# mahdeslami11/jalil-saboorizadeh-Multi-speaker-Neural-Vocoder

Measured on AMD Instinct MI355X. Metric: audio samples/sec gen (3-tier dim1024) + TBPTT steps/sec @1/2/4/8 GPU, higher is better.
Workload: dtype bf16

## Files before the change

### jalil-saboorizadeh-multi-speaker-neural-vocoder_amd/csrc/gru_xcd.hip

```cpp
#include <algorithm>

#include "samplernn_hip_internal.hpp"
#include "handoff.hpp"
#include "gru_point.hpp"

namespace gx {
constexpr int NW = 8, NTHR = NW * 64;
constexpr int RG = 16;
constexpr int CU = 32;
constexpr int NT = 6;
constexpr int UK = 32;
constexpr int MAXMT = 4;
constexpr int PS = 68;
constexpr int HDR = 2048;
}

__device__ __forceinline__ void gx_note_failure(const int* err, int* sticky) {
    if (threadIdx.x == 0) {
        const int e = __hip_atomic_load(err, __ATOMIC_RELAXED, __HIP_MEMORY_SCOPE_AGENT);
        if (e) __hip_atomic_fetch_max(sticky, e, __ATOMIC_RELAXED, __HIP_MEMORY_SCOPE_AGENT);
    }
}

struct GruXArgs {
    const float* gi; int64_t ldgi; int64_t sgi;
    const float* h0;
    const bf16* whh; const float* bhh;
    float* out; bf16* out_lp; int64_t ldo; int64_t so;
    bf16* hp_lp;
    float* gates; int64_t ldg; int64_t sg;
    u64* xh;
    int* census;
    int nolocal;
    int* err;
    int* sticky;
    int spin_limit;
    int withhold;
    int B, D, Fr, G, P, RV;
    int poll_sleep;
    unsigned long long* diag;
    int exp;
};

template <int UPW, int MT, int DC = 0>
__global__ __launch_bounds__(gx::NTHR, 2) void gru_xcd_fwd_kernel(GruXArgs a) {
    using namespace gx;
    extern __shared__ __attribute__((aligned(16))) char smem[];
    const int tid = threadIdx.x, wave = tid >> 6, lane = tid & 63;
    const int D = DC ? DC : a.D, B = a.B, RV = a.RV;
    const int NU = D / UK, KW = NW < NU ? NW : NU;
    float* red = (float*)smem;
    int* gsh = (int*)(smem + (size_t)2 * KW * NT * 4 * PS * sizeof(float));
    const int g = blockIdx.x % a.G, p = blockIdx.x / a.G;
    if (tid == 0) hx_group_arrive(a.census + g * a.P + p);
    const int u0 = p * CU;
    const int DG = D / 2;
    unsigned long long* dg = (a.diag && blockIdx.x == 0 && tid == 0) ? a.diag : nullptr;
    int nd = 0;
#define GX_STAMP() do { if (dg && nd < 255) dg[nd++] = __builtin_amdgcn_s_memrealtime(); } while (0)
    bf16x8 wf[UPW][NT];
    {
        const int PW = 2 * D + 16;
        const int PPR = D / 8;
        char* stg = smem;
        uint4 lw[UPW][NT];
#pragma unroll
        for (int gate = 0; gate < 3; ++gate) {
            if (gate) __syncthreads();
            const bf16* src = a.whh + (int64_t)(gate * D + u0) * D;
            if constexpr (DC != 0) {
                constexpr int NPT = 32 * (DC / 8) / NTHR;
                uint4 v[NPT];
#pragma unroll
                for (int i = 0; i < NPT; ++i) {
                    const int e = tid + i * NTHR, rr = e / PPR, c = e - rr * PPR;
                    v[i] = *reinterpret_cast<const uint4*>(src + (int64_t)rr * D + c * 8);
                }
#pragma unroll
                for (int i = 0; i < NPT; ++i) {
                    const int e = tid + i * NTHR, rr = e / PPR, c = e - rr * PPR;
                    *reinterpret_cast<uint4*>(stg + rr * PW + c * 16) = v[i];
                }
            } else {
                for (int e = tid; e < 32 * PPR; e += NTHR) {
                    const int rr = e / PPR, c = e - rr * PPR;
                    *reinterpret_cast<uint4*>(stg + rr * PW + c * 16) =
                        *reinterpret_cast<const uint4*>(src + (int64_t)rr * D + c * 8);
                }
            }
            __syncthreads();
#pragma unroll
            for (int j = 0; j < UPW; ++j) {
                const int u = wave + NW * j;
                const int ke = min(u * UK + (lane >> 4) * 8, D - 8);
#pragma unroll
                for (int h = 0; h < 2; ++h)
                    lw[j][2 * gate + h] = *reinterpret_cast<const uint4*>(
                        stg + (h * 16 + (lane & 15)) * PW + ke * 2);
            }
        }
        __syncthreads();
#pragma unroll
        for (int j = 0; j < UPW; ++j) {
            const bool kv = wave + NW * j < NU;
#pragma unroll
            for (int t = 0; t < NT; ++t) {
                const uint4 v = kv ? lw[j][t] : make_uint4(0u, 0u, 0u, 0u);
                __builtin_memcpy(&wf[j][t], &v, 16);
            }
        }
    }
    if (wave == 0) {
        const int loc = hx_group_local(a.census + g * a.P, a.P, a.err, !a.nolocal) ? 1 : 0;
        if (tid == 0) gsh[2] = loc;
    }
    __syncthreads();
    const bool local = gsh[2] != 0;
    if (dg) dg[255] = local ? 1 : 2;
    const int r = tid >> 5, uu = tid & 31;
    const bool rv = r < RV;
    const int unit = u0 + uu;
    int rop = r;
    auto row_of = [&](int m) { return (g * MT + m) * RV + rop; };
    const float bhr = a.bhh[unit], bhz = a.bhh[D + unit], bhn = a.bhh[2 * D + unit];
    float hprev[MT];
#pragma unroll
    for (int m = 0; m < MT; ++m) {
        const int row = row_of(m);
        const int b = min(row, B - 1);
        hprev[m] = a.h0[(int64_t)b * D + unit];
        if (a.hp_lp && rv && row < B)
            a.hp_lp[(int64_t)b * a.ldo + unit] = __float2bfloat16(hprev[m]);
    }
    const __amdgpu_buffer_rsrc_t rx = hx_rsrc(a.xh);
    const size_t bufw = (size_t)a.G * MT * RG * DG;
    auto publish = [&](int s, int m, float h) {
        const uint32_t mine = (uint32_t)__bfloat16_as_ushort(__float2bfloat16(h));
        const uint32_t nb = lane_next16(mine);
        if ((uu & 1) == 0 && !(a.withhold && blockIdx.x == 0))
            hx_put(a.xh + ((s + 1) & 1) * bufw + (size_t)(g * MT + m) * RG * DG +
                       ((size_t)(((unit >> 5) * 2 + ((unit & 7) >> 2)) * 64 +
                                 ((unit & 31) >> 3) * 16 + r) << 1) + ((unit & 3) >> 1),
                   (uint32_t)(s + 2), mine | (nb << 16), local);
    };
#pragma unroll
    for (int m = 0; m < MT; ++m) publish(-1, m, hprev[m]);
    const int lrow = lane & 15;
    struct Gi { float r, z, n; };
    Gi ga, gb{0.f, 0.f, 0.f};
    const bool ntl = !(a.exp & 512), nts = !(a.exp & 2048);
    auto ld = [ntl](const float* p) { return ntl ? __builtin_nontemporal_load(p) : *p; };
    {
        const float* gp0 = a.gi + (int64_t)min(row_of(0), B - 1) * a.ldgi;
        ga = Gi{ld(gp0 + unit), ld(gp0 + D + unit), ld(gp0 + 2 * D + unit)};
    }
    auto fetch_gi = [&](int t, int m, Gi& nx) {
        if (a.exp & 2) return;
        int tn = t, mn = m + 1;
        if (mn == MT) { mn = 0; tn = min(t + 1, a.Fr - 1); }
        const float* gp = a.gi + (int64_t)min(row_of(mn), B - 1) * a.ldgi + (int64_t)tn * a.sgi;
        nx.r = ld(gp + unit); nx.z = ld(gp + D + unit); nx.n = ld(gp + 2 * D + unit);
    };
    auto step = [&](int t, int m, const Gi& cu, Gi& nx) {
            floatx4 acc[NT];
    #pragma unroll
            for (int i = 0; i < NT; ++i) acc[i] = floatx4{0.f, 0.f, 0.f, 0.f};
            const bool polls = UPW >= 2 || wave < KW;
            if (!polls) fetch_gi(t, m, nx);
            if (polls) {
                const uint32_t tag = (uint32_t)(t + 1);
                const uint32_t base = (uint32_t)(((size_t)(t & 1) * bufw +
                                                  (size_t)(g * MT + m) * RG * DG) * 8) +
                                      (lrow < RV ? lane * 16u : 0x80000000u);
                uint32_t w[UPW][4];
                int spins = 0;
                for (;;) {
                    uint4 x[UPW][2];
    #pragma unroll
                    for (int j = 0; j < UPW; ++j) {
                        const int u = min(wave + NW * j, NU - 1);
                        const uint32_t off = base + (uint32_t)u * 2048u;
                        x[j][0] = hx_get2(rx, off);
                        x[j][1] = hx_get2(rx, off + 1024);
                    }
                    bool ok = true;
    #pragma unroll
                    for (int j = 0; j < UPW; ++j) {
                        const bool v = wave + NW * j < NU;
                        w[j][0] = v ? x[j][0].x : 0u; w[j][1] = v ? x[j][0].z : 0u;
                        w[j][2] = v ? x[j][1].x : 0u; w[j][3] = v ? x[j][1].z : 0u;
                        ok &= !v || ((x[j][0].y == tag) & (x[j][0].w == tag) &
                                     (x[j][1].y == tag) & (x[j][1].w == tag));
                    }
                    ok |= lrow >= RV;
                    if (__all(ok)) break;
                    if (hx_spin_fail(spins, a.err, lane, a.poll_sleep, a.spin_limit)) break;
                }
                fetch_gi(t, m, nx);
                GX_STAMP();
    #pragma unroll
                for (int j = 0; j < UPW; ++j) {
                    const uint4 v = make_uint4(w[j][0], w[j][1], w[j][2], w[j][3]);
                    bf16x8 af;
                    __builtin_memcpy(&af, &v, 16);
    #pragma unroll
                    for (int i = 0; i < NT; ++i) Mma<bf16>::run(acc[i], af, wf[j][i]);
                }
                float* rb = red + (size_t)(((t * MT + m) & 1) * KW + wave) * NT * 4 * PS + lane;
    #pragma unroll
                for (int i = 0; i < NT; ++i)
    #pragma unroll
                    for (int e = 0; e < 4; ++e) rb[(i * 4 + e) * PS] = acc[i][e];
            }
            GX_STAMP();
            __syncthreads();
            GX_STAMP();
            float gh[3];
            {
                const int ln = (r >> 2) * 16 + (uu & 15), ii = r & 3;
                const float* rb = red + (size_t)((t * MT + m) & 1) * KW * NT * 4 * PS + ii * PS + ln;
    #pragma unroll
                for (int gt = 0; gt < 3; ++gt) {
                    const int tile = 2 * gt + (uu >> 4);
                    float v = 0.f;
                    float pr[NW];
                    #pragma unroll
                    for (int kw = 0; kw < NW; ++kw)
                        pr[kw] = rb[(min(kw, KW - 1) * NT + tile) * 4 * PS];
                    #pragma unroll
                    for (int kw = 0; kw < NW; ++kw) v += kw < KW ? pr[kw] : 0.f;
                    gh[gt] = v;
                }
            }
            const float ghr = gh[0] + bhr, ghz = gh[1] + bhz, ghn = gh[2] + bhn;
            const float rr = 1.0f / (1.0f + expf(-(ghr + cu.r)));
            const float zz = 1.0f / (1.0f + expf(-(ghz + cu.z)));
            const float nn = tanhf(cu.n + ghn * rr);
            const float hn = (hprev[m] - nn) * zz + nn;
            hprev[m] = hn;
            publish(t, m, hn);
            GX_STAMP();
            const int row = row_of(m);
            if (rv && row < B && !(a.exp & 1)) {
                const int64_t o = (int64_t)row * a.ldo + (int64_t)t * a.so + unit;
                float* gt = a.gates + (int64_t)row * a.ldg + (int64_t)t * a.sg;
                const unsigned short hb = __bfloat16_as_ushort(__float2bfloat16(hn));
                unsigned short* olp = reinterpret_cast<unsigned short*>(a.out_lp);
                unsigned short* hlp = reinterpret_cast<unsigned short*>(a.hp_lp);
                if (nts) {
                    __builtin_nontemporal_store(hn, a.out + o);
                    __builtin_nontemporal_store(hb, olp + o);
                    if (a.hp_lp && t + 1 < a.Fr) __builtin_nontemporal_store(hb, hlp + o + a.so);
                    __builtin_nontemporal_store(rr, gt + unit);
                    __builtin_nontemporal_store(zz, gt + D + unit);
                    __builtin_nontemporal_store(nn, gt + 2 * D + unit);
                    __builtin_nontemporal_store(ghn, gt + 3 * D + unit);
                } else {
                    a.out[o] = hn;
                    olp[o] = hb;
                    if (a.hp_lp && t + 1 < a.Fr) hlp[o + a.so] = hb;
                    gt[unit] = rr; gt[D + unit] = zz; gt[2 * D + unit] = nn; gt[3 * D + unit] = ghn;
                }
            }
            GX_STAMP();
    };
    constexpr int TU = MT == 1 ? 2 : 1;
    for (int t0 = 0; t0 < a.Fr; t0 += TU) {
        if (MT > 1) asm volatile("" : "+v"(rop));
#pragma unroll
        for (int q = 0; q < TU * MT; ++q) {
            const int t = t0 + q / MT, m = q % MT;
            if (t >= a.Fr) break;
            if (q & 1) step(t, m, gb, ga);
            else step(t, m, ga, gb);
        }
    }
#undef GX_STAMP
    gx_note_failure(a.err, a.sticky);
}

struct GruXBwdArgs {
    const float* dy; int64_t lddy; int64_t sdy;
    const float* gates; int64_t ldg; int64_t sg;
    const float* hout; int64_t ldo; int64_t so;
    const float* h0;
    const bf16* whh_t;
    float* dgh; bf16* dgh_lp; float* dgi; int64_t ldd; int64_t sd;
    bf16* dgi_lp;
    float* bsum;
    float* ddir0;
    u64* xg;
    int* census;
    int nolocal;
    int* err;
    int* sticky;
    int spin_limit;
    int withhold;
    int B, D, Fr, G, P, RV;
    int exp;
};

template <int UPW, bool FULL, int MT>
__global__ __launch_bounds__(gx::NTHR, 2) void gru_xcd_bwd_kernel(GruXBwdArgs a) {
    using namespace gx;
    extern __shared__ __attribute__((aligned(16))) char smem[];
    const int tid = threadIdx.x, wave = tid >> 6, lane = tid & 63;
    const int D = a.D, B = a.B, K3 = 3 * D, RV = a.RV;
    const int NU = K3 / UK, KW = NW < NU ? NW : NU;
    constexpr int NTB = 2;
    float* red = (float*)smem;
    const size_t red_bytes = (size_t)2 * KW * NTB * 4 * PS * sizeof(float);
    int* gsh = (int*)(smem + red_bytes);
    const int g = blockIdx.x % a.G, p = blockIdx.x / a.G;
    if (tid == 0) hx_group_arrive(a.census + g * a.P + p);
    const int u0 = p * CU;
    const int KG = K3 / 2;
    bf16x8 wf[UPW][NTB];
    {
        uint4 lw[UPW][NTB];
#pragma unroll
        for (int j = 0; j < UPW; ++j) {
            const int u = wave + NW * j;
            const int ke = min(u * UK + (lane >> 4) * 8, K3 - 8);
#pragma unroll
            for (int t = 0; t < NTB; ++t) {
                const int row = u0 + t * 16 + (lane & 15);
                lw[j][t] = *reinterpret_cast<const uint4*>(a.whh_t + (int64_t)row * K3 + ke);
            }
        }
#pragma unroll
        for (int j = 0; j < UPW; ++j) {
            const bool kv = wave + NW * j < NU;
#pragma unroll
            for (int t = 0; t < NTB; ++t) {
                const uint4 v = kv ? lw[j][t] : make_uint4(0u, 0u, 0u, 0u);
                __builtin_memcpy(&wf[j][t], &v, 16);
            }
        }
    }
    if (wave == 0) {
        const int loc = hx_group_local(a.census + g * a.P, a.P, a.err, !a.nolocal) ? 1 : 0;
        if (tid == 0) gsh[2] = loc;
    }
    __syncthreads();
    const bool local = gsh[2] != 0;
    const int r = tid >> 5, uu = tid & 31;
    const bool rv = r < RV;
    const int unit = u0 + uu;
    int rop = r;
    auto row_of = [&](int m) { return (g * MT + m) * RV + rop; };
    const __amdgpu_buffer_rsrc_t rx = hx_rsrc(a.xg);
    const size_t bufw = (size_t)a.G * MT * RG * KG;
    const int lrow = lane & 15;
    auto fetch = [&](int t, int m, float& dyv, float& gr, float& gz, float& gn, float& gg,
                     float& hp) {
        const int b = min(row_of(m), B - 1);
        dyv = a.dy[(int64_t)b * a.lddy + (int64_t)t * a.sdy + unit];
        const float* gp = a.gates + (int64_t)b * a.ldg + (int64_t)t * a.sg;
        gr = gp[unit]; gz = gp[D + unit]; gn = gp[2 * D + unit]; gg = gp[3 * D + unit];
        hp = t > 0 ? a.hout[(int64_t)b * a.ldo + (int64_t)(t - 1) * a.so + unit]
                   : a.h0[(int64_t)b * D + unit];
    };
    float dyv, gr, gz, gn, gg, hp;
    float ddir1 = 0.f, sar1 = 0.f, saz1 = 0.f, sghn1 = 0.f, san1 = 0.f;
    float* sl = (float*)(smem + red_bytes + 64);
    if (MT > 1)
        for (int k = 0; k < 5 * MT; ++k) sl[k * NTHR + tid] = 0.f;
    fetch(a.Fr - 1, 0, dyv, gr, gz, gn, gg, hp);
    for (int t = a.Fr - 1; t >= 0; --t) {
    asm volatile("" : "+v"(rop));
#pragma unroll 1
    for (int m = 0; m < MT; ++m) {
        const bool has_next = t + 1 < a.Fr;
        float* q = sl + (m * 5) * NTHR + tid;
        const float ddir_in = MT == 1 ? ddir1 : q[0];
        floatx4 acc[NTB];
#pragma unroll
        for (int i = 0; i < NTB; ++i) acc[i] = floatx4{0.f, 0.f, 0.f, 0.f};
        if (has_next) {
            if (UPW >= 2 || wave < KW) {
                const uint32_t tag = (uint32_t)(a.Fr - 1 - t);
                const uint32_t base = (uint32_t)((((size_t)((t + 1) & 1)) * bufw +
                                                  (size_t)((g * MT + m) * RG + lrow) * KG) * 8);
                uint4 x[UPW][2];
                int spins = 0;
                uint32_t lb = (uint32_t)((wave * UK + (lane >> 4) * 8) / 2) * 8u;
                asm volatile("" : "+v"(lb));
                for (;;) {
                    if (a.exp & 32) {
#pragma unroll
                        for (int j = 0; j < UPW; ++j)
                            x[j][0] = x[j][1] = make_uint4(lane, tag, lane, tag);
                        asm volatile("" : "+v"(x[0][0].x));
                        break;
                    }
#pragma unroll
                    for (int j = 0; j < UPW; ++j) {
                        const int u = min(wave + NW * j, NU - 1);
                        const uint32_t off =
                            FULL ? base + lb + (uint32_t)(j * NW * UK / 2 * 8)
                                 : base + (uint32_t)((u * UK + (lane >> 4) * 8) / 2) * 8u;
                        x[j][0] = hx_get2(rx, off);
                        x[j][1] = hx_get2(rx, off + 16);
                    }
                    if (a.exp & 8) break;
                    bool ok = true;
#pragma unroll
                    for (int j = 0; j < UPW; ++j)
                        ok &= (wave + NW * j >= NU) ||
                              ((x[j][0].y == tag) & (x[j][0].w == tag) & (x[j][1].y == tag) &
                               (x[j][1].w == tag));
                    if (__all(ok)) break;
                    if (hx_spin_fail(spins, a.err, lane, 1, a.spin_limit)) break;
                }
#pragma unroll
                for (int j = 0; j < UPW; ++j) {
                    const bool kv = wave + NW * j < NU;
                    const uint4 v = kv ? make_uint4(x[j][0].x, x[j][0].z, x[j][1].x, x[j][1].z)
                                       : make_uint4(0u, 0u, 0u, 0u);
                    bf16x8 af;
                    __builtin_memcpy(&af, &v, 16);
                    if (a.exp & 4) {
                        asm volatile("" :: "v"(v.x), "v"(v.y), "v"(v.z), "v"(v.w));
                        continue;
                    }
#pragma unroll
                    for (int i = 0; i < NTB; ++i) Mma<bf16>::run(acc[i], af, wf[j][i]);
                }
                float* rb = red + (size_t)((((a.Fr - 1 - t) * MT + m) & 1) * KW + wave) * NTB * 4 * PS + lane;
#pragma unroll
                for (int i = 0; i < NTB; ++i)
#pragma unroll
                    for (int e = 0; e < 4; ++e) rb[(i * 4 + e) * PS] = acc[i][e];
            }
            if (!(a.exp & 16)) __syncthreads();
        }
        float s = 0.f;
        if (has_next) {
            const int ln = (r >> 2) * 16 + (uu & 15), ii = r & 3, tile = uu >> 4;
            const float* rb = red + (size_t)(((a.Fr - 1 - t) * MT + m) & 1) * KW * NTB * 4 * PS +
                              ii * PS + ln;
            float pr[NW];
#pragma unroll
            for (int kw = 0; kw < NW; ++kw) pr[kw] = rb[(min(kw, KW - 1) * NTB + tile) * 4 * PS];
#pragma unroll
            for (int kw = 0; kw < NW; ++kw) s += kw < KW ? pr[kw] : 0.f;
        }
        float dh = s + dyv;
        if (has_next) dh += ddir_in;
        const GruBwdPoint o = gru_bwd_point(dh, gr, gz, gn, gg, hp);
        if (MT == 1) ddir1 = o.ddir;
        else q[0] = o.ddir;
        {
            const float vals[3] = {o.dar, o.daz, o.dghn};
            u64* dst = a.xg + (size_t)(t & 1) * bufw + (size_t)((g * MT + m) * RG + r) * KG;
#pragma unroll
            for (int gt = 0; gt < 3; ++gt) {
                const uint32_t mine = (uint32_t)__bfloat16_as_ushort(__float2bfloat16(vals[gt]));
                const uint32_t nb = lane_next16(mine);
                if ((uu & 1) == 0 && !(a.withhold && blockIdx.x == 0))
                    hx_put(dst + (gt * D + unit) / 2, (uint32_t)(a.Fr - t), mine | (nb << 16), local);
            }
        }
        const float cdar = o.dar, cdaz = o.daz, cdghn = o.dghn, cdan = o.dan;
        if (!(a.exp & 2)) {
            if (m + 1 < MT) fetch(t, m + 1, dyv, gr, gz, gn, gg, hp);
            else if (t > 0) fetch(t - 1, 0, dyv, gr, gz, gn, gg, hp);
        }
        const int row = row_of(m);
        if (rv && row < B && !(a.exp & 1)) {
            const int64_t ob = (int64_t)row * a.ldd + (int64_t)t * a.sd;
            if (a.dgh) {
                float* dg = a.dgh + ob;
                dg[unit] = cdar; dg[D + unit] = cdaz; dg[2 * D + unit] = cdghn;
            }
            bf16* dl = a.dgh_lp + ob;
            const bf16 har = __float2bfloat16(cdar), haz = __float2bfloat16(cdaz);
            dl[unit] = har; dl[D + unit] = haz; dl[2 * D + unit] = __float2bfloat16(cdghn);
            if (a.dgi) {
                float* di = a.dgi + ob;
                di[unit] = cdar; di[D + unit] = cdaz; di[2 * D + unit] = cdan;
            }
            if (a.dgi_lp) {
                bf16* dj = a.dgi_lp + ob;
                dj[unit] = har; dj[D + unit] = haz; dj[2 * D + unit] = __float2bfloat16(cdan);
            }
            if (MT == 1) {
                sar1 += cdar; saz1 += cdaz; sghn1 += cdghn; san1 += cdan;
            } else {
                q[NTHR] += cdar; q[2 * NTHR] += cdaz; q[3 * NTHR] += cdghn; q[4 * NTHR] += cdan;
            }
            if (t == 0) a.ddir0[(int64_t)row * D + unit] = o.ddir;
        }
    }
    }
#pragma unroll
    for (int m = 0; m < MT; ++m) {
        const int row = row_of(m);
        if (a.bsum && rv && row < B) {
            float* bs = a.bsum + (int64_t)row * 4 * D;
            if (MT == 1) {
                bs[unit] = sar1; bs[D + unit] = saz1; bs[2 * D + unit] = sghn1;
                bs[3 * D + unit] = san1;
            } else {
                const float* q = sl + (m * 5) * NTHR + tid;
                bs[unit] = q[NTHR]; bs[D + unit] = q[2 * NTHR]; bs[2 * D + unit] = q[3 * NTHR];
                bs[3 * D + unit] = q[4 * NTHR];
            }
        }
    }
    gx_note_failure(a.err, a.sticky);
}

template <int UPW, int MT>
__global__ __launch_bounds__(gx::NTHR, 2) void gru_xcd_bwd_pk_kernel(GruXBwdArgs a) {
    using namespace gx;
    extern __shared__ __attribute__((aligned(16))) char smem[];
    const int tid = threadIdx.x, wave = tid >> 6, lane = tid & 63;
    constexpr int D = UPW * 64;
    const int B = a.B, RV = a.RV;
    constexpr int KW = NW;
    constexpr int NTB = 2;
    float* red = (float*)smem;
    const size_t red_bytes = (size_t)2 * KW * NTB * 4 * PS * sizeof(float);
    int* gsh = (int*)(smem + red_bytes);
    const int g = blockIdx.x % a.G, p = blockIdx.x / a.G;
    if (tid == 0) hx_group_arrive(a.census + g * a.P + p);
    const int u0 = p * CU;
    bf16x8 wf[UPW][NTB];
    {
        constexpr int PW = 2 * D + 16;
        constexpr int PPR = D / 8;
        constexpr int NPT = 32 * PPR / NTHR;
        static_assert((32 * PPR) % NTHR == 0, "gru_xcd_bwd_pk: staging split");
        char* stg = smem;
        unsigned lr[UPW][NTB], lz[UPW][NTB], ln[UPW][NTB];
        auto stage = [&](int gt, unsigned (&lw)[UPW][NTB]) __attribute__((always_inline)) {
            if (gt) __syncthreads();
#pragma unroll
            for (int i = 0; i < NPT; ++i) {
                const int e = tid + i * NTHR, rr = e / PPR, c = e - rr * PPR;
                *reinterpret_cast<uint4*>(stg + rr * PW + c * 16) =
                    *reinterpret_cast<const uint4*>(a.whh_t + (int64_t)(u0 + rr) * 3 * D +
                                                    gt * D + c * 8);
            }
            __syncthreads();
#pragma unroll
            for (int j = 0; j < UPW; ++j) {
                const int iu = (wave + NW * j) * 8 + (lane >> 4) * 2;
#pragma unroll
                for (int t = 0; t < NTB; ++t)
                    lw[j][t] = *reinterpret_cast<const unsigned*>(
                        stg + (t * 16 + (lane & 15)) * PW + iu * 2);
            }
        };
        stage(0, lr);
        stage(1, lz);
        stage(2, ln);
        __syncthreads();
#pragma unroll
        for (int j = 0; j < UPW; ++j)
#pragma unroll
            for (int t = 0; t < NTB; ++t) {
                const unsigned r2 = lr[j][t], z2 = lz[j][t], n2 = ln[j][t];
                const uint4 v = make_uint4((r2 & 0xffffu) | (z2 << 16), n2 & 0xffffu,
                                           (r2 >> 16) | (z2 & 0xffff0000u), n2 >> 16);
                __builtin_memcpy(&wf[j][t], &v, 16);
            }
    }
    if (wave == 0) {
        const int loc = hx_group_local(a.census + g * a.P, a.P, a.err, !a.nolocal) ? 1 : 0;
        if (tid == 0) gsh[2] = loc;
    }
    __syncthreads();
    const bool local = gsh[2] != 0;
    const int r = tid >> 5, uu = tid & 31;
    const bool rv = r < RV;
    const int unit = u0 + uu;
    int rop = r;
    auto row_of = [&](int m) { return (g * MT + m) * RV + rop; };
    const __amdgpu_buffer_rsrc_t rx = hx_rsrc(a.xg);
    const size_t bufw = (size_t)a.G * MT * RG * D;
    const int lrow = lane & 15;
    const __amdgpu_buffer_rsrc_t rdy = hx_rsrc(a.dy), rgt = hx_rsrc(a.gates),
                                 rho = hx_rsrc(a.hout), rh0 = hx_rsrc(a.h0);
    const bool plain = (a.exp & 512) != 0;
    auto ldf = [plain](__amdgpu_buffer_rsrc_t r, uint32_t off) {
        return __uint_as_float(plain ? __builtin_amdgcn_raw_buffer_load_b32(r, off, 0, 0)
                                     : __builtin_amdgcn_raw_buffer_load_b32(r, off, 0, 2 ));
    };
    auto fetch = [&](int t, int m, float& dyv, float& gr, float& gz, float& gn, float& gg,
                     float& hp) {
        const uint32_t b = (uint32_t)min(row_of(m), B - 1);
        dyv = ldf(rdy, (uint32_t)(b * a.lddy + t * a.sdy + unit) * 4u);
        const uint32_t go = (uint32_t)(b * a.ldg + t * a.sg + unit) * 4u;
        gr = ldf(rgt, go); gz = ldf(rgt, go + 4u * D); gn = ldf(rgt, go + 8u * D);
        gg = ldf(rgt, go + 12u * D);
        hp = t > 0 ? ldf(rho, (uint32_t)(b * a.ldo + (t - 1) * a.so + unit) * 4u)
                   : ldf(rh0, (uint32_t)(b * D + unit) * 4u);
    };
    float dyv, gr, gz, gn, gg, hp;
    float ddir1 = 0.f, sar1 = 0.f, saz1 = 0.f, sghn1 = 0.f, san1 = 0.f;
    float* sl = (float*)(smem + red_bytes + 64);
    if (MT > 1)
        for (int k = 0; k < 5 * MT; ++k) sl[k * NTHR + tid] = 0.f;
    fetch(a.Fr - 1, 0, dyv, gr, gz, gn, gg, hp);
    for (int t = a.Fr - 1; t >= 0; --t) {
    asm volatile("" : "+v"(rop));
#pragma unroll 1
    for (int m = 0; m < MT; ++m) {
        const bool has_next = t + 1 < a.Fr;
        float* q = sl + (m * 5) * NTHR + tid;
        const float ddir_in = MT == 1 ? ddir1 : q[0];
        floatx4 acc[NTB];
#pragma unroll
        for (int i = 0; i < NTB; ++i) acc[i] = floatx4{0.f, 0.f, 0.f, 0.f};
        if (has_next) {
            const uint32_t tag = (uint32_t)(a.Fr - 1 - t);
            const uint32_t base = (uint32_t)((((size_t)((t + 1) & 1)) * bufw +
                                              (size_t)(g * MT + m) * RG * D) * 8);
            uint4 x[UPW];
            int spins = 0;
            uint32_t lb = lrow < RV ? (uint32_t)(wave * 64 + lane) * 16u : 0x80000000u;
            asm volatile("" : "+v"(lb));
            for (;;) {
#pragma unroll
                for (int j = 0; j < UPW; ++j)
                    x[j] = hx_get2(rx, base + lb + (uint32_t)(j * NW * 64 * 16));
                bool ok = true;
#pragma unroll
                for (int j = 0; j < UPW; ++j)
                    ok &= ((x[j].y >> 16) == tag) & ((x[j].w >> 16) == tag);
                ok |= lrow >= RV;
                if (__all(ok)) break;
                if (hx_spin_fail(spins, a.err, lane, 1, a.spin_limit)) break;
            }
#pragma unroll
            for (int j = 0; j < UPW; ++j) {
                bf16x8 af;
                __builtin_memcpy(&af, &x[j], 16);
#pragma unroll
                for (int i = 0; i < NTB; ++i) Mma<bf16>::run(acc[i], af, wf[j][i]);
            }
            float* rb = red + (size_t)((((a.Fr - 1 - t) * MT + m) & 1) * KW + wave) * NTB * 4 * PS + lane;
#pragma unroll
            for (int i = 0; i < NTB; ++i)
#pragma unroll
                for (int e = 0; e < 4; ++e) rb[(i * 4 + e) * PS] = acc[i][e];
            __syncthreads();
        }
        float s = 0.f;
        if (has_next) {
            const int ln = (r >> 2) * 16 + (uu & 15), ii = r & 3, tile = uu >> 4;
            const float* rb = red + (size_t)(((a.Fr - 1 - t) * MT + m) & 1) * KW * NTB * 4 * PS +
                              ii * PS + ln;
            float pr[NW];
#pragma unroll
            for (int kw = 0; kw < NW; ++kw) pr[kw] = rb[(kw * NTB + tile) * 4 * PS];
#pragma unroll
            for (int kw = 0; kw < NW; ++kw) s += pr[kw];
        }
        float dh = s + dyv;
        if (has_next) dh += ddir_in;
        const GruBwdPoint o = gru_bwd_point(dh, gr, gz, gn, gg, hp);
        if (MT == 1) ddir1 = o.ddir;
        else q[0] = o.ddir;
        if (!(a.withhold && blockIdx.x == 0)) {
            u64* dst = a.xg + (size_t)(t & 1) * bufw + (size_t)(g * MT + m) * RG * D +
                       ((size_t)((unit >> 3) * 64 + ((unit & 7) >> 1) * 16 + r) << 1) + (unit & 1);
            const u64 v = (u64)__bfloat16_as_ushort(__float2bfloat16(o.dar)) |
                          ((u64)__bfloat16_as_ushort(__float2bfloat16(o.daz)) << 16) |
                          ((u64)__bfloat16_as_ushort(__float2bfloat16(o.dghn)) << 32) |
                          ((u64)(uint32_t)(a.Fr - t) << 48);
            if (local) __hip_atomic_store(dst, v, __ATOMIC_RELAXED, __HIP_MEMORY_SCOPE_WORKGROUP);
            else __hip_atomic_store(dst, v, __ATOMIC_RELAXED, __HIP_MEMORY_SCOPE_AGENT);
        }
        const float cdar = o.dar, cdaz = o.daz, cdghn = o.dghn, cdan = o.dan;
        if (!(a.exp & 64)) {
            if (m + 1 < MT) fetch(t, m + 1, dyv, gr, gz, gn, gg, hp);
            else if (t > 0) fetch(t - 1, 0, dyv, gr, gz, gn, gg, hp);
        }
        const int row = row_of(m);
        if (rv && row < B && !(a.exp & 1)) {
            const int64_t ob = (int64_t)row * a.ldd + (int64_t)t * a.sd;
            if (a.dgh) {
                float* dg = a.dgh + ob;
                dg[unit] = cdar; dg[D + unit] = cdaz; dg[2 * D + unit] = cdghn;
            }
            unsigned short* dl = reinterpret_cast<unsigned short*>(a.dgh_lp + ob);
            const unsigned short har = __bfloat16_as_ushort(__float2bfloat16(cdar)),
                                 haz = __bfloat16_as_ushort(__float2bfloat16(cdaz)),
                                 hgn = __bfloat16_as_ushort(__float2bfloat16(cdghn)),
                                 han = __bfloat16_as_ushort(__float2bfloat16(cdan));
            const bool nts = !(a.exp & 2048);
            if (nts) {
                __builtin_nontemporal_store(har, dl + unit);
                __builtin_nontemporal_store(haz, dl + D + unit);
                __builtin_nontemporal_store(hgn, dl + 2 * D + unit);
            } else {
                dl[unit] = har; dl[D + unit] = haz; dl[2 * D + unit] = hgn;
            }
            if (a.dgi) {
                float* di = a.dgi + ob;
                di[unit] = cdar; di[D + unit] = cdaz; di[2 * D + unit] = cdan;
            }
            if (a.dgi_lp) {
                unsigned short* dj = reinterpret_cast<unsigned short*>(a.dgi_lp + ob);
                if (nts) {
                    __builtin_nontemporal_store(har, dj + unit);
                    __builtin_nontemporal_store(haz, dj + D + unit);
                    __builtin_nontemporal_store(han, dj + 2 * D + unit);
                } else {
                    dj[unit] = har; dj[D + unit] = haz; dj[2 * D + unit] = han;
                }
            }
            if (MT == 1) {
                sar1 += cdar; saz1 += cdaz; sghn1 += cdghn; san1 += cdan;
            } else {
                q[NTHR] += cdar; q[2 * NTHR] += cdaz; q[3 * NTHR] += cdghn; q[4 * NTHR] += cdan;
            }
            if (t == 0) a.ddir0[(int64_t)row * D + unit] = o.ddir;
        }
    }
    }
#pragma unroll
    for (int m = 0; m < MT; ++m) {
        const int row = row_of(m);
        if (a.bsum && rv && row < B) {
            float* bs = a.bsum + (int64_t)row * 4 * D;
            if (MT == 1) {
                bs[unit] = sar1; bs[D + unit] = saz1; bs[2 * D + unit] = sghn1;
                bs[3 * D + unit] = san1;
            } else {
                const float* q = sl + (m * 5) * NTHR + tid;
                bs[unit] = q[NTHR]; bs[D + unit] = q[2 * NTHR]; bs[2 * D + unit] = q[3 * NTHR];
                bs[3 * D + unit] = q[4 * NTHR];
            }
        }
    }
    gx_note_failure(a.err, a.sticky);
}


static unsigned long long*& gx_diag_buf() {
    static unsigned long long* p = nullptr;
    return p;
}

extern "C" int srnn_gru_diag_dump(void) {
    unsigned long long h[256];
    if (!gx_diag_buf() || hipDeviceSynchronize() != hipSuccess ||
        hipMemcpy(h, gx_diag_buf(), sizeof(h), hipMemcpyDeviceToHost) != hipSuccess)
        return 1;
    fprintf(stderr, "gru_xcd diag mode: %s\n", h[255] == 1 ? "xcd-local" : "static map");
    for (int k = 1; k < 255 && h[k]; ++k)
        fprintf(stderr, "gru_xcd diag %3d: +%8.2f us\n", k, (double)(h[k] - h[k - 1]) / 100.0);
    return 0;
}

static int gx_cus() {
    return srnn_device_cus() / srnn_device_share();
}

struct GxLayout { int mt, G, rv, P; };

static int gx_launch_rows(int D) {
    const int ncu = gx_cus();
    if (ncu <= 0 || D % 256 != 0 || D > 1024) return 0;
    return (ncu / (D / gx::CU)) * gx::RG * gx::MAXMT;
}

static bool gx_layout(int B, int D, GxLayout& L) {
    const int ncu = gx_cus();
    if (ncu <= 0 || B <= 0 || D % 256 != 0 || D > 1024) return false;
    L.P = D / gx::CU;
    const int gmax = ncu / L.P;
    if (gmax < 1) return false;
    L.mt = 1;
    while (L.mt < gx::MAXMT && cdiv(B, gx::RG * L.mt) > gmax) L.mt *= 2;
    int G = cdiv(B, gx::RG * L.mt);
    if (G > gmax) return false;
    L.G = (G + 7) / 8 * 8 <= gmax ? (G + 7) / 8 * 8 : G;
    L.rv = cdiv(B, L.G * L.mt);
    return L.rv <= gx::RG;
}

extern "C" size_t srnn_gru_xcd_work_bytes(int dtype, int B, int D) {
    if (dtype != SRNN_BF16 || B <= 0) return 0;
    const int lr = gx_launch_rows(D);
    GxLayout L;
    if (lr <= 0 || !gx_layout(B < lr ? B : lr, D, L)) return 0;
    return gx::HDR + (size_t)2 * L.G * L.mt * gx::RG * (D / 2) * 8;
}

extern "C" int srnn_gru_xcd_fwd2(int dtype, int B, int D, int Fr, const float* gi, int64_t ldgi,
                                 int64_t sgi, const float* h0, const void* whh, const float* bhh,
                                 float* out, void* out_lp, int64_t ldo, int64_t so, float* gates,
                                 int64_t ldg, int64_t sg, void* hprev_lp, void* work,
                                 size_t work_bytes, void* stream) {
    const size_t need = srnn_gru_xcd_work_bytes(dtype, B, D);
    SRNN_REQUIRE(need > 0, "gru_xcd: shape/device not supported");
    SRNN_REQUIRE(work && work_bytes >= need, "gru_xcd: workspace %zu < %zu", work_bytes, need);
    if (Fr <= 0) return 0;
    const int lr = gx_launch_rows(D);
    if (B > lr) {
        for (int c = 0; c < B; c += lr) {
            const int n = B - c < lr ? B - c : lr;
            const int rc = srnn_gru_xcd_fwd2(
                dtype, n, D, Fr, gi + (int64_t)c * ldgi, ldgi, sgi, h0 + (int64_t)c * D, whh,
                bhh, out + (int64_t)c * ldo, (bf16*)out_lp + (int64_t)c * ldo, ldo, so,
                gates + (int64_t)c * ldg, ldg, sg,
                hprev_lp ? (void*)((bf16*)hprev_lp + (int64_t)c * ldo) : nullptr, work,
                work_bytes, stream);
            if (rc) return rc;
        }
        return 0;
    }
    GxLayout L;
    SRNN_REQUIRE(gx_layout(B, D, L), "gru_xcd: no row layout for B=%d D=%d", B, D);
    hipStream_t s = (hipStream_t)stream;
    SRNN_CHECK_HIP(hipMemsetAsync(work, 0, need, s));
    GruXArgs a;
    a.gi = gi; a.ldgi = ldgi; a.sgi = sgi;
    a.h0 = h0; a.whh = (const bf16*)whh; a.bhh = bhh;
    a.out = out; a.out_lp = (bf16*)out_lp; a.ldo = ldo; a.so = so;
    a.hp_lp = (bf16*)hprev_lp;
    a.gates = gates; a.ldg = ldg; a.sg = sg;
    a.err = (int*)work;
    a.sticky = srnn_sticky_flag();
    SRNN_REQUIRE(a.sticky, "gru_xcd: sticky flag allocation failed");
    a.spin_limit = srnn_persist_spin_limit(hx::SPIN_LIMIT);
    a.withhold = env_flag("SRNN_PERSIST_FORCE_FAIL", 0);
    a.census = (int*)work + 16;
    a.nolocal = !env_flag("SRNN_GEN_LOCAL", 1);
    a.xh = (u64*)((char*)work + gx::HDR);
    a.B = B; a.D = D; a.Fr = Fr;
    a.diag = nullptr;
    a.poll_sleep = env_flag("SRNN_POLL_SLEEP", 1);
    a.exp = env_flag("SRNN_GX_EXP", 0);
    {
        static unsigned long long* diag = nullptr;
        static int armed = -1;
        if (armed < 0) armed = env_flag("SRNN_GRU_DIAG", 0);
        if (armed == 1 && Fr >= 32 && hipMalloc(&diag, 256 * 8) == hipSuccess) {
            SRNN_CHECK_HIP(hipMemsetAsync(diag, 0, 256 * 8, s));
            a.diag = diag;
            armed = 2;
            gx_diag_buf() = diag;
        }
    }
    a.G = L.G;
    a.P = L.P;
    a.RV = L.rv;
    const int NU = D / gx::UK;
    const int KW = NU < gx::NW ? NU : gx::NW;
    const size_t lds = (size_t)2 * KW * gx::NT * 4 * gx::PS * 4 + 16;
    const int upw = cdiv(NU, gx::NW);
    const int ui = upw <= 1 ? 0 : upw <= 2 ? 1 : 2;
    const int mi = L.mt == 1 ? 0 : L.mt == 2 ? 1 : 2;
    typedef void (*FwdK)(GruXArgs);
    static const FwdK ks[3][3] = {
        {gru_xcd_fwd_kernel<1, 1>, gru_xcd_fwd_kernel<1, 2>, gru_xcd_fwd_kernel<1, 4>},
        {gru_xcd_fwd_kernel<2, 1>, gru_xcd_fwd_kernel<2, 2>, gru_xcd_fwd_kernel<2, 4>},
        {gru_xcd_fwd_kernel<4, 1>, gru_xcd_fwd_kernel<4, 2>, gru_xcd_fwd_kernel<4, 4>}};
    static const FwdK k1024[3] = {gru_xcd_fwd_kernel<4, 1, 1024>, gru_xcd_fwd_kernel<4, 2, 1024>,
                                  gru_xcd_fwd_kernel<4, 4, 1024>};
    const FwdK k = D == 1024 && env_flag("SRNN_GX_DC", 1) ? k1024[mi] : ks[ui][mi];
    static bool attr[4][3] = {};
    const int ai = k == ks[ui][mi] ? ui : 3;
    if (!attr[ai][mi]) {
        SRNN_CHECK_HIP(hipFuncSetAttribute((const void*)k,
                                           hipFuncAttributeMaxDynamicSharedMemorySize,
                                           160 * 1024));
        attr[ai][mi] = true;
    }
    if (srnn_persist_check((const void*)k, gx::NTHR, lds, (int64_t)a.G * a.P, "gru_xcd_fwd"))
        return 1;
    hipLaunchKernelGGL(k, dim3(a.G * a.P), dim3(gx::NTHR), lds, s, a);
    SRNN_LAUNCH_CHECK();
    return 0;
}

extern "C" int srnn_gru_xcd_fwd(int dtype, int B, int D, int Fr, const float* gi, int64_t ldgi,
                                int64_t sgi, const float* h0, const void* whh, const float* bhh,
                                float* out, void* out_lp, int64_t ldo, int64_t so, float* gates,
                                int64_t ldg, int64_t sg, void* work, size_t work_bytes,
                                void* stream) {
    return srnn_gru_xcd_fwd2(dtype, B, D, Fr, gi, ldgi, sgi, h0, whh, bhh, out, out_lp, ldo, so,
                             gates, ldg, sg, nullptr, work, work_bytes, stream);
}


extern "C" size_t srnn_gru_xcd_bwd_work_bytes(int dtype, int B, int D) {
    if (!srnn_gru_xcd_work_bytes(dtype, B, D)) return 0;
    const int lr = gx_launch_rows(D);
    GxLayout L;
    if (!gx_layout(B < lr ? B : lr, D, L)) return 0;
    return gx::HDR + (size_t)2 * L.G * L.mt * gx::RG * (3 * D / 2) * 8;
}

extern "C" int srnn_gru_xcd_bwd2(int dtype, int B, int D, int Fr, const float* dy, int64_t lddy,
                                 int64_t sdy, const float* gates, int64_t ldg, int64_t sg,
                                 const float* hout, int64_t ldo, int64_t so, const float* h0,
                                 const void* whh_t, float* dgh, void* dgh_lp, float* dgi,
                                 void* dgi_lp, float* bsum, int64_t ldd, int64_t sd, float* ddir0,
                                 void* work, size_t work_bytes, void* stream) {
    const size_t need = srnn_gru_xcd_bwd_work_bytes(dtype, B, D);
    SRNN_REQUIRE(need > 0, "gru_xcd_bwd: shape/device not supported");
    SRNN_REQUIRE(work && work_bytes >= need, "gru_xcd_bwd: workspace %zu < %zu", work_bytes, need);
    SRNN_REQUIRE(dgh_lp, "gru_xcd_bwd: dgh_lp is required");
    if (Fr <= 0) return 0;
    const int lr = gx_launch_rows(D);
    if (B > lr) {
        for (int c = 0; c < B; c += lr) {
            const int n = B - c < lr ? B - c : lr;
            const int rc = srnn_gru_xcd_bwd2(
                dtype, n, D, Fr, dy + (int64_t)c * lddy, lddy, sdy, gates + (int64_t)c * ldg,
                ldg, sg, hout + (int64_t)c * ldo, ldo, so, h0 + (int64_t)c * D, whh_t,
                dgh ? dgh + (int64_t)c * ldd : nullptr, (bf16*)dgh_lp + (int64_t)c * ldd,
                dgi ? dgi + (int64_t)c * ldd : nullptr,
                dgi_lp ? (void*)((bf16*)dgi_lp + (int64_t)c * ldd) : nullptr,
                bsum ? bsum + (int64_t)c * 4 * D : nullptr, ldd, sd, ddir0 + (int64_t)c * D,
                work, work_bytes, stream);
            if (rc) return rc;
        }
        return 0;
    }
    GxLayout L;
    SRNN_REQUIRE(gx_layout(B, D, L), "gru_xcd_bwd: no row layout for B=%d D=%d", B, D);
    hipStream_t s = (hipStream_t)stream;
    const int64_t omax = std::max({((int64_t)(B - 1) * lddy + (int64_t)(Fr - 1) * sdy + D) * 4,
                                   ((int64_t)(B - 1) * ldg + (int64_t)(Fr - 1) * sg + 4 * D) * 4,
                                   ((int64_t)(B - 1) * ldo + (int64_t)(Fr - 1) * so + D) * 4,
                                   (int64_t)B * D * 4});
    const bool pk = D % 64 == 0 && D / 64 <= 16 && (D / 64) % 4 == 0 && Fr < 0x7f80 &&
                    omax < 0x7fffffffll - 64 && env_flag("SRNN_GX_PK", 1);
    const size_t clear = pk ? gx::HDR + (size_t)2 * L.G * L.mt * gx::RG * D * 8 : need;
    SRNN_CHECK_HIP(hipMemsetAsync(work, 0, clear, s));
    GruXBwdArgs a;
    a.dy = dy; a.lddy = lddy; a.sdy = sdy;
    a.gates = gates; a.ldg = ldg; a.sg = sg;
    a.hout = hout; a.ldo = ldo; a.so = so; a.h0 = h0;
    a.whh_t = (const bf16*)whh_t;
    a.dgh = dgh; a.dgh_lp = (bf16*)dgh_lp; a.dgi = dgi; a.ldd = ldd; a.sd = sd;
    a.dgi_lp = (bf16*)dgi_lp; a.bsum = bsum;
    a.ddir0 = ddir0;
    a.err = (int*)work;
    a.sticky = srnn_sticky_flag();
    SRNN_REQUIRE(a.sticky, "gru_xcd_bwd: sticky flag allocation failed");
    a.spin_limit = srnn_persist_spin_limit(hx::SPIN_LIMIT);
    a.withhold = env_flag("SRNN_PERSIST_FORCE_FAIL", 0);
    a.census = (int*)work + 16;
    a.nolocal = !env_flag("SRNN_GEN_LOCAL", 1);
    a.xg = (u64*)((char*)work + gx::HDR);
    a.B = B; a.D = D; a.Fr = Fr;
    a.exp = env_flag("SRNN_GX_EXP", 0);
    a.G = L.G;
    a.P = L.P;
    a.RV = L.rv;
    const int NU = 3 * D / gx::UK;
    const int KW = pk ? gx::NW : NU < gx::NW ? NU : gx::NW;
    size_t lds = (size_t)2 * KW * 2 * 4 * gx::PS * 4 + 64 +
                 (L.mt > 1 ? (size_t)L.mt * 5 * gx::NTHR * 4 : 0);
    if (pk) {
        const size_t stage = (size_t)32 * (2 * D + 16);
        if (lds < stage) lds = stage;
        typedef void (*PkK)(GruXBwdArgs);
        static const PkK kp[4][3] = {
            {gru_xcd_bwd_pk_kernel<4, 1>, gru_xcd_bwd_pk_kernel<4, 2>, gru_xcd_bwd_pk_kernel<4, 4>},
            {gru_xcd_bwd_pk_kernel<8, 1>, gru_xcd_bwd_pk_kernel<8, 2>, gru_xcd_bwd_pk_kernel<8, 4>},
            {gru_xcd_bwd_pk_kernel<12, 1>, gru_xcd_bwd_pk_kernel<12, 2>,
             gru_xcd_bwd_pk_kernel<12, 4>},
            {gru_xcd_bwd_pk_kernel<16, 1>, gru_xcd_bwd_pk_kernel<16, 2>,
             gru_xcd_bwd_pk_kernel<16, 4>}};
        const int mi = L.mt == 1 ? 0 : L.mt == 2 ? 1 : 2;
        const PkK k = kp[D / 256 - 1][mi];
        static bool attr[4][3] = {};
        if (!attr[D / 256 - 1][mi]) {
            SRNN_CHECK_HIP(hipFuncSetAttribute((const void*)k,
                                               hipFuncAttributeMaxDynamicSharedMemorySize,
                                               160 * 1024));
            attr[D / 256 - 1][mi] = true;
        }
        if (srnn_persist_check((const void*)k, gx::NTHR, lds, (int64_t)a.G * a.P, "gru_xcd_bwd"))
            return 1;
        hipLaunchKernelGGL(k, dim3(a.G * a.P), dim3(gx::NTHR), lds, s, a);
        SRNN_LAUNCH_CHECK();
        return 0;
    }
    const int upw = cdiv(NU, gx::NW);
    const int ui = upw <= 3 ? 0 : upw <= 6 ? 1 : 2;
    const bool full = NU == (ui == 0 ? 3 : ui == 1 ? 6 : 12) * gx::NW;
    const int mi = L.mt == 1 ? 0 : L.mt == 2 ? 1 : 2;
    typedef void (*BwdK)(GruXBwdArgs);
    static const BwdK ks[2][3][3] = {
        {{nullptr, nullptr, nullptr},
         {nullptr, nullptr, nullptr},
         {gru_xcd_bwd_kernel<12, false, 1>, gru_xcd_bwd_kernel<12, false, 2>,
          gru_xcd_bwd_kernel<12, false, 4>}},
        {{gru_xcd_bwd_kernel<3, true, 1>, gru_xcd_bwd_kernel<3, true, 2>,
          gru_xcd_bwd_kernel<3, true, 4>},
         {gru_xcd_bwd_kernel<6, true, 1>, gru_xcd_bwd_kernel<6, true, 2>,
          gru_xcd_bwd_kernel<6, true, 4>},
         {gru_xcd_bwd_kernel<12, true, 1>, gru_xcd_bwd_kernel<12, true, 2>,
          gru_xcd_bwd_kernel<12, true, 4>}}};
    const BwdK k = ks[full ? 1 : 0][ui][mi];
    SRNN_REQUIRE(k, "gru_xcd_bwd: no kernel for D=%d", D);
    if (srnn_persist_check((const void*)k, gx::NTHR, lds, (int64_t)a.G * a.P, "gru_xcd_bwd"))
        return 1;
    hipLaunchKernelGGL(k, dim3(a.G * a.P), dim3(gx::NTHR), lds, s, a);
    SRNN_LAUNCH_CHECK();
    return 0;
}

extern "C" int srnn_gru_xcd_bwd(int dtype, int B, int D, int Fr, const float* dy, int64_t lddy,
                                int64_t sdy, const float* gates, int64_t ldg, int64_t sg,
                                const float* hout, int64_t ldo, int64_t so, const float* h0,
                                const void* whh_t, float* dgh, void* dgh_lp, float* dgi,
                                int64_t ldd, int64_t sd, float* ddir0, void* work,
                                size_t work_bytes, void* stream) {
    return srnn_gru_xcd_bwd2(dtype, B, D, Fr, dy, lddy, sdy, gates, ldg, sg, hout, ldo, so, h0,
                             whh_t, dgh, dgh_lp, dgi, nullptr, nullptr, ldd, sd, ddir0, work,
                             work_bytes, stream);
}

extern "C" int srnn_gru_xcd_error(const void* work) {
    int e = 0;
    if (hipMemcpy(&e, work, sizeof(int), hipMemcpyDeviceToHost) != hipSuccess) return -1;
    return e;
}
```

Measured before the change: 39.89 million.

## Batch two row tiles per barrier in packed GRU backward kernel

Adds a BT=2 variant of the packed GRU backward persistent kernel that handles two M-tiles per step. It polls and runs the MMAs for both tiles, takes a single __syncthreads, then reduces, publishes and stores both, with the next pair's inputs prefetched in between. This halves the number of block-wide barriers and reduction round trips per timestep and lets the two tiles' work overlap. In exchange it doubles the LDS reduction buffer, which may lower occupancy, and adds register pressure. The variant is on by default through SRNN_GX_BATCH whenever MT is 2 or 4.

```diff
diff --git a/jalil-saboorizadeh-multi-speaker-neural-vocoder_amd/csrc/gru_xcd.hip b/jalil-saboorizadeh-multi-speaker-neural-vocoder_amd/csrc/gru_xcd.hip
--- a/jalil-saboorizadeh-multi-speaker-neural-vocoder_amd/csrc/gru_xcd.hip
+++ b/jalil-saboorizadeh-multi-speaker-neural-vocoder_amd/csrc/gru_xcd.hip
@@ -512,7 +512,7 @@
     gx_note_failure(a.err, a.sticky);
 }
 
-template <int UPW, int MT>
+template <int UPW, int MT, int BT = 1>
 __global__ __launch_bounds__(gx::NTHR, 2) void gru_xcd_bwd_pk_kernel(GruXBwdArgs a) {
     using namespace gx;
     extern __shared__ __attribute__((aligned(16))) char smem[];
@@ -522,7 +522,7 @@
     constexpr int KW = NW;
     constexpr int NTB = 2;
     float* red = (float*)smem;
-    const size_t red_bytes = (size_t)2 * KW * NTB * 4 * PS * sizeof(float);
+    const size_t red_bytes = (size_t)2 * BT * KW * NTB * 4 * PS * sizeof(float);
     int* gsh = (int*)(smem + red_bytes);
     const int g = blockIdx.x % a.G, p = blockIdx.x / a.G;
     if (tid == 0) hx_group_arrive(a.census + g * a.P + p);
@@ -605,6 +605,147 @@
     if (MT > 1)
         for (int k = 0; k < 5 * MT; ++k) sl[k * NTHR + tid] = 0.f;
     fetch(a.Fr - 1, 0, dyv, gr, gz, gn, gg, hp);
+    if constexpr (BT == 2) {
+    static_assert(MT % 2 == 0, "gru_xcd_bwd_pk: a batch is two tiles");
+    float dy1, gr1, gz1, gn1, gg1, hp1;
+    fetch(a.Fr - 1, 1, dy1, gr1, gz1, gn1, gg1, hp1);
+    auto poll_mma = [&](int t, int m, int par, int k) {
+        floatx4 acc[NTB];
+#pragma unroll
+        for (int i = 0; i < NTB; ++i) acc[i] = floatx4{0.f, 0.f, 0.f, 0.f};
+        const uint32_t tag = (uint32_t)(a.Fr - 1 - t);
+        const uint32_t base = (uint32_t)((((size_t)((t + 1) & 1)) * bufw +
+                                          (size_t)(g * MT + m) * RG * D) * 8);
+        uint4 x[UPW];
+        int spins = 0;
+        uint32_t lb = lrow < RV ? (uint32_t)(wave * 64 + lane) * 16u : 0x80000000u;
+        asm volatile("" : "+v"(lb));
+        for (;;) {
+#pragma unroll
+            for (int j = 0; j < UPW; ++j)
+                x[j] = hx_get2(rx, base + lb + (uint32_t)(j * NW * 64 * 16));
+            bool ok = true;
+#pragma unroll
+            for (int j = 0; j < UPW; ++j)
+                ok &= ((x[j].y >> 16) == tag) & ((x[j].w >> 16) == tag);
+            ok |= lrow >= RV;
+            if (__all(ok)) break;
+            if (hx_spin_fail(spins, a.err, lane, 1, a.spin_limit)) break;
+        }
+#pragma unroll
+        for (int j = 0; j < UPW; ++j) {
+            bf16x8 af;
+            __builtin_memcpy(&af, &x[j], 16);
+#pragma unroll
+            for (int i = 0; i < NTB; ++i) Mma<bf16>::run(acc[i], af, wf[j][i]);
+        }
+        float* rb = red + (size_t)((par * 2 + k) * KW + wave) * NTB * 4 * PS + lane;
+#pragma unroll
+        for (int i = 0; i < NTB; ++i)
+#pragma unroll
+            for (int e = 0; e < 4; ++e) rb[(i * 4 + e) * PS] = acc[i][e];
+    };
+    auto reduce = [&](int par, int k) {
+        const int ln = (r >> 2) * 16 + (uu & 15), ii = r & 3, tile = uu >> 4;
+        const float* rb = red + (size_t)(par * 2 + k) * KW * NTB * 4 * PS + ii * PS + ln;
+        float pr[NW], s = 0.f;
+#pragma unroll
+        for (int kw = 0; kw < NW; ++kw) pr[kw] = rb[(kw * NTB + tile) * 4 * PS];
+#pragma unroll
+        for (int kw = 0; kw < NW; ++kw) s += pr[kw];
+        return s;
+    };
+    uint32_t pslot = ((uint32_t)((unit >> 3) * 64 + ((unit & 7) >> 1) * 16 + r) << 1) + (unit & 1);
+    auto publish = [&](int t, int m, const GruBwdPoint& o) {
+        if (!(a.withhold && blockIdx.x == 0)) {
+            u64* dst = a.xg + (size_t)(t & 1) * bufw + (size_t)(g * MT + m) * RG * D + pslot;
+            const u64 v = (u64)__bfloat16_as_ushort(__float2bfloat16(o.dar)) |
+                          ((u64)__bfloat16_as_ushort(__float2bfloat16(o.daz)) << 16) |
+                          ((u64)__bfloat16_as_ushort(__float2bfloat16(o.dghn)) << 32) |
+                          ((u64)(uint32_t)(a.Fr - t) << 48);
+            if (local) __hip_atomic_store(dst, v, __ATOMIC_RELAXED, __HIP_MEMORY_SCOPE_WORKGROUP);
+            else __hip_atomic_store(dst, v, __ATOMIC_RELAXED, __HIP_MEMORY_SCOPE_AGENT);
+        }
+    };
+    auto store = [&](int t, int m, float cdar, float cdaz, float cdghn, float cdan, float cddir,
+                     float* q) {
+        const int row = row_of(m);
+        if (rv && row < B && !(a.exp & 1)) {
+            const int64_t ob = (int64_t)row * a.ldd + (int64_t)t * a.sd;
+            if (a.dgh) {
+                float* dg = a.dgh + ob;
+                dg[unit] = cdar; dg[D + unit] = cdaz; dg[2 * D + unit] = cdghn;
+            }
+            unsigned short* dl = reinterpret_cast<unsigned short*>(a.dgh_lp + ob);
+            const unsigned short har = __bfloat16_as_ushort(__float2bfloat16(cdar)),
+                                 haz = __bfloat16_as_ushort(__float2bfloat16(cdaz)),
+                                 hgn = __bfloat16_as_ushort(__float2bfloat16(cdghn)),
+                                 han = __bfloat16_as_ushort(__float2bfloat16(cdan));
+            const bool nts = !(a.exp & 2048);
+            if (nts) {
+                __builtin_nontemporal_store(har, dl + unit);
+                __builtin_nontemporal_store(haz, dl + D + unit);
+                __builtin_nontemporal_store(hgn, dl + 2 * D + unit);
+            } else {
+                dl[unit] = har; dl[D + unit] = haz; dl[2 * D + unit] = hgn;
+            }
+            if (a.dgi) {
+                float* di = a.dgi + ob;
+                di[unit] = cdar; di[D + unit] = cdaz; di[2 * D + unit] = cdan;
+            }
+            if (a.dgi_lp) {
+                unsigned short* dj = reinterpret_cast<unsigned short*>(a.dgi_lp + ob);
+                if (nts) {
+                    __builtin_nontemporal_store(har, dj + unit);
+                    __builtin_nontemporal_store(haz, dj + D + unit);
+                    __builtin_nontemporal_store(han, dj + 2 * D + unit);
+                } else {
+                    dj[unit] = har; dj[D + unit] = haz; dj[2 * D + unit] = han;
+                }
+            }
+            q[NTHR] += cdar; q[2 * NTHR] += cdaz; q[3 * NTHR] += cdghn; q[4 * NTHR] += cdan;
+            if (t == 0) a.ddir0[(int64_t)row * D + unit] = cddir;
+        }
+    };
+    for (int t = a.Fr - 1; t >= 0; --t) {
+    asm volatile("" : "+v"(rop), "+v"(pslot));
+#pragma unroll 1
+    for (int m0 = 0; m0 < MT; m0 += 2) {
+        const bool has_next = t + 1 < a.Fr;
+        float* q0 = sl + (m0 * 5) * NTHR + tid;
+        float* q1 = q0 + 5 * NTHR;
+        const int par = ((a.Fr - 1 - t) * (MT / 2) + m0 / 2) & 1;
+        float s0 = 0.f, s1 = 0.f;
+        if (has_next) {
+            poll_mma(t, m0, par, 0);
+            poll_mma(t, m0 + 1, par, 1);
+            __syncthreads();
+            s0 = reduce(par, 0);
+            s1 = reduce(par, 1);
+        }
+        float dh0 = s0 + dyv, dh1 = s1 + dy1;
+        if (has_next) { dh0 += q0[0]; dh1 += q1[0]; }
+        const GruBwdPoint o0 = gru_bwd_point(dh0, gr, gz, gn, gg, hp);
+        const GruBwdPoint o1 = gru_bwd_point(dh1, gr1, gz1, gn1, gg1, hp1);
+        q0[0] = o0.ddir;
+        q1[0] = o1.ddir;
+        publish(t, m0, o0);
+        publish(t, m0 + 1, o1);
+        if (!(a.exp & 64)) {
+            if (m0 + 2 < MT) {
+                fetch(t, m0 + 2, dyv, gr, gz, gn, gg, hp);
+                fetch(t, m0 + 3, dy1, gr1, gz1, gn1, gg1, hp1);
+            } else if (t > 0) {
+                fetch(t - 1, 0, dyv, gr, gz, gn, gg, hp);
+                fetch(t - 1, 1, dy1, gr1, gz1, gn1, gg1, hp1);
+            }
+        }
+        store(t, m0, o0.dar, o0.daz, o0.dghn, o0.dan, o0.ddir, q0);
+        store(t, m0 + 1, o1.dar, o1.daz, o1.dghn, o1.dan, o1.ddir, q1);
+    }
+    }
+    rop = r;
+    } else {
     for (int t = a.Fr - 1; t >= 0; --t) {
     asm volatile("" : "+v"(rop));
 #pragma unroll 1
@@ -721,6 +862,7 @@
             }
             if (t == 0) a.ddir0[(int64_t)row * D + unit] = o.ddir;
         }
+    }
     }
     }
 #pragma unroll
@@ -973,14 +1115,21 @@
              gru_xcd_bwd_pk_kernel<12, 4>},
             {gru_xcd_bwd_pk_kernel<16, 1>, gru_xcd_bwd_pk_kernel<16, 2>,
              gru_xcd_bwd_pk_kernel<16, 4>}};
+        static const PkK kpb[4][3] = {
+            {nullptr, gru_xcd_bwd_pk_kernel<4, 2, 2>, gru_xcd_bwd_pk_kernel<4, 4, 2>},
+            {nullptr, gru_xcd_bwd_pk_kernel<8, 2, 2>, gru_xcd_bwd_pk_kernel<8, 4, 2>},
+            {nullptr, gru_xcd_bwd_pk_kernel<12, 2, 2>, gru_xcd_bwd_pk_kernel<12, 4, 2>},
+            {nullptr, gru_xcd_bwd_pk_kernel<16, 2, 2>, gru_xcd_bwd_pk_kernel<16, 4, 2>}};
         const int mi = L.mt == 1 ? 0 : L.mt == 2 ? 1 : 2;
-        const PkK k = kp[D / 256 - 1][mi];
-        static bool attr[4][3] = {};
-        if (!attr[D / 256 - 1][mi]) {
+        const int bi = kpb[D / 256 - 1][mi] && env_flag("SRNN_GX_BATCH", 1) ? 1 : 0;
+        const PkK k = bi ? kpb[D / 256 - 1][mi] : kp[D / 256 - 1][mi];
+        if (bi) lds += (size_t)2 * KW * 2 * 4 * gx::PS * 4;
+        static bool attr[2][4][3] = {};
+        if (!attr[bi][D / 256 - 1][mi]) {
             SRNN_CHECK_HIP(hipFuncSetAttribute((const void*)k,
                                                hipFuncAttributeMaxDynamicSharedMemorySize,
                                                160 * 1024));
-            attr[D / 256 - 1][mi] = true;
+            attr[bi][D / 256 - 1][mi] = true;
         }
         if (srnn_persist_check((const void*)k, gx::NTHR, lds, (int64_t)a.G * a.P, "gru_xcd_bwd"))
             return 1;
```

Result: faster. 40.44 million (median of 6 runs) (+1.4%).
